# noway/nzcp-circom

Hardware: NVIDIA B200
Metric: groth16_proofs_per_sec (higher is better)
Workload: dtype u256 (Fr/Fq Montgomery, 8x32-bit limbs, IMAD.WIDE carry chains)

## Files before the change

nzcp_circom_b200/csrc/msm.cu:

```cuda
#include <atomic>

#include "common.cuh"
#include "msm_pair.cuh"

#ifndef NZCP_G2_ACC_BLOCKS
#define NZCP_G2_ACC_BLOCKS 3
#endif

namespace nzcp {

#ifndef NZCP_TASK_LEN_MAX
#define NZCP_TASK_LEN_MAX 64
#endif
static constexpr int kTaskLenMax = NZCP_TASK_LEN_MAX;
static_assert((NZCP_TASK_LEN_MAX & (NZCP_TASK_LEN_MAX - 1)) == 0 && NZCP_TASK_LEN_MAX >= 8, "task length must be a power of two");
static constexpr int kTaskLenMin = 8;
#ifndef NZCP_TARGET_TASKS
#define NZCP_TARGET_TASKS (148 * 640)
#endif
static constexpr int kTargetTasks = NZCP_TARGET_TASKS;
#ifndef NZCP_HEAVY_TASKS
#define NZCP_HEAVY_TASKS 16
#endif
static constexpr int kHeavyTasks = NZCP_HEAVY_TASKS;
// ... 275 lines not shown
#pragma unroll
  for (int r = 0; r < C; r++) carry[r] = 0;
  for (uint32_t base = 0; base < n_buckets; base += 4096) {
    const uint32_t b0 = base + threadIdx.x * 4;
    uint32_t v[C][4], sum[C], incl[C];
#pragma unroll
    for (int r = 0; r < C; r++) sum[r] = 0;
#pragma unroll
    for (int k = 0; k < 4; k++) {
      const uint32_t b = b0 + k;
      uint32_t len = b < n_buckets ? offsets[(size_t)(b + 1) * n_copies] - offsets[(size_t)b * n_copies] : 0u;
#pragma unroll
      for (int r = 0; r < C; r++) {
        v[r][k] = len;
        sum[r] += len;
        len = (len + 1) >> 1;
      }
      if (b < n_buckets) red_count[b] = v[R][k];
    }
#pragma unroll
    for (int r = 0; r < C; r++) {
      incl[r] = sum[r];
#pragma unroll
      for (int d = 1; d < 32; d <<= 1) {
        const uint32_t y = __shfl_up_sync(0xffffffffu, incl[r], d);
        if (lane >= (uint32_t)d) incl[r] += y;
      }
      if (lane == 31) wsum[r][warp] = incl[r];
    }
    __syncthreads();
    if (warp < (uint32_t)C) {
      const uint32_t w = wsum[warp][lane];
      uint32_t z = w;
#pragma unroll
      for (int d = 1; d < 32; d <<= 1) {
        const uint32_t y = __shfl_up_sync(0xffffffffu, z, d);
        if (lane >= (uint32_t)d) z += y;
      }
      wsum[warp][lane] = z - w;
      if (lane == 31) chunk_total[warp] = z;
    }
    __syncthreads();
#pragma unroll
    for (int r = 0; r < C; r++) {
      uint32_t run = carry[r] + wsum[r][warp] + (incl[r] - sum[r]);
#pragma unroll
      for (int k = 0; k < 4; k++) {
        if (b0 + k < n_buckets) round_off[(size_t)r * pitch + b0 + k] = run;
        run += v[r][k];
      }
      carry[r] += chunk_total[r];
    }
    __syncthreads();
  }
  if (threadIdx.x == 0) {
#pragma unroll
    for (int r = 0; r < C; r++) round_off[(size_t)r * pitch + n_buckets] = carry[r];
    flags[5] = carry[R];
  }
}

__global__ void __launch_bounds__(256)
msm_task_fill_kernel(const uint32_t* __restrict__ bcount, const uint32_t* __restrict__ offsets,
                     const uint32_t* __restrict__ task_off, uint2* __restrict__ tasks, uint32_t n_buckets,
                     const uint32_t* __restrict__ flags) {
  const uint32_t t = blockIdx.x * blockDim.x + threadIdx.x;
  if (t >= flags[2]) return;
  const uint32_t tl = flags[4];
  uint32_t lo = 0, hi = n_buckets;
  while (hi - lo > 1) {
    uint32_t mid = (lo + hi) >> 1;
    if (task_off[mid] <= t) lo = mid; else hi = mid;
  }
  (void)tl;
  const uint32_t k = task_off[lo + 1] - task_off[lo], j = t - task_off[lo];
  const uint32_t cnt = bcount[lo], base = cnt / k, rem = cnt % k;
  tasks[t] = make_uint2(offsets[lo] + j * base + (j < rem ? j : rem), base + (j < rem ? 1u : 0u));
}

template <class T>
__device__ __forceinline__ void prefetch_l1(const T* p) {
  asm volatile("prefetch.global.L1 [%0];" ::"l"(p));
  if (sizeof(T) > 64) asm volatile("prefetch.global.L1 [%0];" ::"l"(reinterpret_cast<const char*>(p) + 64));
}

template <class F> struct AccumOcc { static constexpr int kBlocks = 5; };
template <> struct AccumOcc<Fq2> { static constexpr int kBlocks = NZCP_G2_ACC_BLOCKS; };

template <class F>
__global__ void __launch_bounds__(128, AccumOcc<F>::kBlocks)
msm_accumulate_kernel(const Affine<F>* __restrict__ table, const uint32_t* __restrict__ entries,
                      const uint2* __restrict__ tasks, const uint32_t* __restrict__ flags, XYZZ<F>* __restrict__ partial, int pf) {
  uint32_t t = blockIdx.x * blockDim.x + threadIdx.x;
  if (t >= flags[2]) return;
  uint2 tk = tasks[t];
  XYZZ<F> acc = XYZZ<F>::inf();
  uint32_t e = entries[tk.x];
  if (pf & 1) prefetch_l1(table + (e & 0x7fffffffu));
  for (uint32_t k = 0; k < tk.y; k++) {
    uint32_t en = e;
    if (k + 1 < tk.y) {
      en = entries[tk.x + k + 1];
      if (pf & 1) prefetch_l1(table + (en & 0x7fffffffu));
    }
    Affine<F> q;
#if defined(__CUDA_ARCH__)
    if (sizeof(F) == sizeof(Fq) && (pf & 4)) q = gather_hinted<Affine<F>>(table + (e & 0x7fffffffu));
    else
#endif
      q = table[e & 0x7fffffffu];
    if (!q.is_inf()) xyzz_madd(acc, q, (e >> 31) != 0);
    e = en;
  }
  partial[t] = acc;
}

template <class F>
__global__ void __launch_bounds__(128, AccumOcc<F>::kBlocks)
msm_accumulate_pts_kernel(const Affine<F>* __restrict__ pts, const uint2* __restrict__ tasks,
                          const uint32_t* __restrict__ flags, XYZZ<F>* __restrict__ partial) {
  uint32_t t = blockIdx.x * blockDim.x + threadIdx.x;
  if (t >= flags[2]) return;
  uint2 tk = tasks[t];
  XYZZ<F> acc = XYZZ<F>::inf();
  for (uint32_t k = 0; k < tk.y; k++) {
    Affine<F> q = pts[tk.x + k];
    if (!q.is_inf()) xyzz_madd(acc, q, false);
  }
  partial[t] = acc;
}

static constexpr int kPairInvGroup = 32;
#ifndef NZCP_PAIR_FWD_BLOCKS
#define NZCP_PAIR_FWD_BLOCKS 1
#endif
template <class F, bool FROM_TABLE, int K>
__global__ void __launch_bounds__(128, (sizeof(F) == sizeof(Fq) ? NZCP_PAIR_FWD_BLOCKS : 1))
msm_pair_forward_kernel(const Affine<F>* __restrict__ src, const uint32_t* __restrict__ entries,
                        const uint32_t* __restrict__ off_in, const uint32_t* __restrict__ off_out, uint32_t n_buckets,
                        F* __restrict__ scratch, F* __restrict__ prod, int pf, Affine<F>* __restrict__ ops) {
  const uint32_t t = blockIdx.x * blockDim.x + threadIdx.x;
  PairSource<F, FROM_TABLE> ps{src, entries, pf};
  msm_pair_forward_body<F, FROM_TABLE, K>(t, gridDim.x * blockDim.x, ps, off_in, off_out, n_buckets, scratch, prod, ops);
}

template <class F, int K>
__global__ void __launch_bounds__(64)
msm_pair_invert_kernel(F* __restrict__ prod, const uint32_t* __restrict__ off_out, uint32_t n_buckets) {
  const uint32_t n_out = off_out[n_buckets];
  const uint32_t n_prod = pair_n_prod<K>(n_out);
  msm_pair_invert_body<F, kPairInvGroup>(blockIdx.x * blockDim.x + threadIdx.x, prod, n_prod);
}

template <class F, bool FROM_TABLE, int K>
__global__ void __launch_bounds__(128)
msm_pair_backward_kernel(const Affine<F>* __restrict__ src, const uint32_t* __restrict__ entries,
                         const uint32_t* __restrict__ off_in, const uint32_t* __restrict__ off_out, uint32_t n_buckets,
                         Affine<F>* __restrict__ dst, const F* __restrict__ scratch, const F* __restrict__ inv_prod, int pf,
                         const Affine<F>* __restrict__ ops) {
  const uint32_t t = blockIdx.x * blockDim.x + threadIdx.x;
  PairSource<F, FROM_TABLE> ps{src, entries, pf};
  msm_pair_backward_body<F, FROM_TABLE, K>(t, gridDim.x * blockDim.x, ps, off_in, off_out, n_buckets, dst, scratch, inv_prod,
                                           ops);
}

template <class T>
__device__ __forceinline__ T load_cg(const T* p) {
  static_assert(sizeof(T) % 16 == 0, "16-byte granules");
  T r;
  const uint4* s = reinterpret_cast<const uint4*>(p);
  uint4* d = reinterpret_cast<uint4*>(&r);
#pragma unroll
  for (int i = 0; i < (int)(sizeof(T) / 16); i++) d[i] = __ldcg(s + i);
  return r;
}

template <class T>
__device__ __forceinline__ T shfl_down_obj(const T& v, unsigned delta) {
  T r;
  const uint32_t* s = reinterpret_cast<const uint32_t*>(&v);
  uint32_t* d = reinterpret_cast<uint32_t*>(&r);
#pragma unroll
  for (int i = 0; i < (int)(sizeof(T) / 4); i++) d[i] = __shfl_down_sync(0xffffffffu, s[i], delta);
  return r;
}

template <class F>
__global__ void __launch_bounds__(128)
msm_combine_kernel(const uint32_t* __restrict__ task_off, const XYZZ<F>* __restrict__ partial,
                   XYZZ<F>* __restrict__ buckets, uint32_t n_buckets, uint32_t* __restrict__ heavy_list,
                   uint32_t* __restrict__ heavy_count) {
  const uint32_t b = blockIdx.x * blockDim.x + threadIdx.x;
  if (b >= n_buckets) return;
  const uint32_t t0 = task_off[b], nt = task_off[b + 1] - t0;
  if (nt > (uint32_t)kHeavyTasks) {
    heavy_list[atomicAdd(heavy_count, 1u)] = b;
    return;
  }
  XYZZ<F> acc = XYZZ<F>::inf();
  for (uint32_t j = 0; j < nt; j++) xyzz_add(acc, partial[t0 + j]);
  buckets[b] = acc;
}

__global__ void __launch_bounds__(1024)
msm_heavy_scan_kernel(const uint32_t* __restrict__ task_off, const uint32_t* __restrict__ heavy_list,
                      uint32_t* __restrict__ heavy_count, uint32_t* __restrict__ chunk_off) {
  __shared__ uint32_t sums[1024];
  const uint32_t n = heavy_count[0];
  const uint32_t per = (n + 1023) / 1024;
  const uint32_t b = threadIdx.x * per;
  const uint32_t e = b + per < n ? b + per : n;
  auto chunks = [&](uint32_t h) {
    uint32_t bk = heavy_list[h];
    return (task_off[bk + 1] - task_off[bk] + kHeavyChunk - 1) / kHeavyChunk;
  };
  uint32_t acc = 0;
  for (uint32_t h = b; h < e; h++) acc += chunks(h);
  sums[threadIdx.x] = acc;
  __syncthreads();
  for (int off = 1; off < 1024; off <<= 1) {
    uint32_t v = threadIdx.x >= (uint32_t)off ? sums[threadIdx.x - off] : 0;
    __syncthreads();
    sums[threadIdx.x] += v;
    __syncthreads();
  }
  uint32_t run = threadIdx.x ? sums[threadIdx.x - 1] : 0;
  for (uint32_t h = b; h < e; h++) {
    chunk_off[h] = run;
    run += chunks(h);
  }
  if (threadIdx.x == 1023) {
    chunk_off[n] = sums[1023];
    heavy_count[1] = sums[1023];
  }
}

template <class F>
__device__ __forceinline__ XYZZ<F> block_sum(XYZZ<F> acc, XYZZ<F>* sm) {
  sm[threadIdx.x] = acc;
  __syncthreads();
  for (uint32_t stride = blockDim.x / 2; stride >= 1; stride >>= 1) {
    if (threadIdx.x < stride) {
      XYZZ<F> a = sm[threadIdx.x];
      xyzz_add(a, sm[threadIdx.x + stride]);
      sm[threadIdx.x] = a;
    }
    __syncthreads();
  }
  XYZZ<F> r = sm[0];
  __syncthreads();
  return r;
}

template <class F>
__global__ void __launch_bounds__(kHeavyThreads)
msm_combine_heavy_kernel(const uint32_t* __restrict__ task_off, const XYZZ<F>* __restrict__ partial,
                         const uint32_t* __restrict__ heavy_list, const uint32_t* __restrict__ heavy_count,
                         const uint32_t* __restrict__ chunk_off, XYZZ<F>* __restrict__ chunk_partial,
                         XYZZ<F>* __restrict__ buckets) {
  extern __shared__ unsigned char heavy_sm_raw[];
  XYZZ<F>* sm = reinterpret_cast<XYZZ<F>*>(heavy_sm_raw);
  const uint32_t n_heavy = *heavy_count;
  const uint32_t total = chunk_off[n_heavy];
  for (uint32_t ch = blockIdx.x; ch < total; ch += gridDim.x) {
    uint32_t lo = 0, hi = n_heavy;
    while (hi - lo > 1) {
      uint32_t mid = (lo + hi) >> 1;
      if (chunk_off[mid] <= ch) lo = mid; else hi = mid;
    }
    const uint32_t b = heavy_list[lo];
    const uint32_t c = ch - chunk_off[lo];
    const uint32_t t0 = task_off[b] + c * kHeavyChunk;
    const uint32_t left = task_off[b + 1] - t0;
    const uint32_t cnt = left < (uint32_t)kHeavyChunk ? left : (uint32_t)kHeavyChunk;
    XYZZ<F> acc = XYZZ<F>::inf();
    for (uint32_t j = threadIdx.x; j < cnt; j += blockDim.x) xyzz_add(acc, partial[t0 + j]);
    acc = block_sum(acc, sm);
    if (threadIdx.x == 0) {
      if (chunk_off[lo + 1] - chunk_off[lo] == 1) buckets[b] = acc;
      else chunk_partial[ch] = acc;
    }
  }
}

template <class F>
__global__ void __launch_bounds__(kHeavyThreads)
msm_combine_heavy2_kernel(const uint32_t* __restrict__ heavy_list, const uint32_t* __restrict__ heavy_count,
                          const uint32_t* __restrict__ chunk_off, const XYZZ<F>* __restrict__ chunk_partial,
                          XYZZ<F>* __restrict__ buckets) {
  extern __shared__ unsigned char heavy_sm_raw[];
  XYZZ<F>* sm = reinterpret_cast<XYZZ<F>*>(heavy_sm_raw);
  const uint32_t n_heavy = *heavy_count;
  for (uint32_t h = blockIdx.x; h < n_heavy; h += gridDim.x) {
    const uint32_t c0 = chunk_off[h], nc = chunk_off[h + 1] - c0;
    if (nc <= 1) continue;
    XYZZ<F> acc = XYZZ<F>::inf();
    for (uint32_t j = threadIdx.x; j < nc; j += blockDim.x) xyzz_add(acc, chunk_partial[c0 + j]);
    acc = block_sum(acc, sm);
    if (threadIdx.x == 0) buckets[heavy_list[h]] = acc;
  }
}

static constexpr int kMargThreads = 128;

template <class F>
__device__ __forceinline__ XYZZ<F> warp_weighted_sum(XYZZ<F> run, uint32_t lane, XYZZ<F>* total) {
  for (uint32_t d = 1; d < 32; d <<= 1) {
    XYZZ<F> o = shfl_down_obj(run, d);
    if (lane + d < 32) xyzz_add(run, o);
  }
  *total = run;
  XYZZ<F> leaf = lane >= 1 ? run : XYZZ<F>::inf();
  for (uint32_t off = 16; off >= 1; off >>= 1) {
    XYZZ<F> o = shfl_down_obj(leaf, off);
    xyzz_add(leaf, o);
  }
// ... 187 lines not shown

void msm_sort_create(MsmSort* s, size_t n_points, int c, int rounds, bool table_free) {
  *s = MsmSort();
  if (c < 2 || c > 20) throw std::runtime_error("msm: window size out of range");
  s->n_points = n_points;
  s->c = c;
  s->rounds = rounds < 0 ? msm_pick_rounds(n_points, c) : (rounds > kMsmMaxRounds ? kMsmMaxRounds : rounds);
  s->n_windows = msm_num_windows(c);
  s->table_free = table_free;
  s->n_groups = table_free ? s->n_windows : 1;
  s->group_buckets = (size_t)1 << (c - 1);
  s->n_buckets = s->group_buckets * s->n_groups;
  if (s->n_buckets > ((size_t)1 << 19)) throw std::runtime_error("msm: too many buckets (window size too large for the table-free path)");
  size_t max_entries = (size_t)s->n_windows * n_points;
  if (max_entries >= ((size_t)1 << 31)) throw std::runtime_error("msm: too many points");
  size_t by_len = max_entries / kTaskLenMax, by_target = 2 * (size_t)kTargetTasks;
  if (max_entries / kTaskLenMin < by_target) by_target = max_entries / kTaskLenMin;
  s->max_tasks = s->n_buckets + (by_len > by_target ? by_len : by_target) + 1;
  size_t tot = 0;
  s->smem_hist = s->n_buckets <= (size_t)kSmemHistBuckets;
  s->n_copies = s->smem_hist ? 148 : kCopiesGlobal;
  size_t n_ctr = s->n_buckets * s->n_copies;
  s->counts = dev_alloc<uint32_t>(n_ctr + 1, &tot);
  s->offsets = dev_alloc<uint32_t>(n_ctr + 1, &tot);
  s->cursors = dev_alloc<uint32_t>(n_ctr + 1, &tot);
  s->red_count = dev_alloc<uint32_t>(s->n_buckets + 1, &tot);
  s->round_off = dev_alloc<uint32_t>((size_t)(kMsmMaxRounds + 1) * (s->n_buckets + 1), &tot);
  s->round_max[0] = max_entries;
  for (int r = 1; r <= kMsmMaxRounds; r++) s->round_max[r] = (s->round_max[r - 1] + s->n_buckets) / 2 + 1;
  s->block_sums = dev_alloc<uint32_t>(2 * (n_ctr / kScanBlock + 2), &tot);
  if (s->smem_hist) {
    NZCP_CUDA(cudaFuncSetAttribute(msm_digits_smem_kernel<false>, cudaFuncAttributeMaxDynamicSharedMemorySize, kSmemHistBuckets * 4));
    NZCP_CUDA(cudaFuncSetAttribute(msm_digits_smem_kernel<true>, cudaFuncAttributeMaxDynamicSharedMemorySize, kSmemHistBuckets * 4));
  }
  s->entries = dev_alloc<uint32_t>(max_entries, &tot);
  s->task_off = dev_alloc<uint32_t>(s->n_buckets + 1, &tot);
  s->tasks = dev_alloc<uint2>(s->max_tasks, &tot);
  s->flags = dev_alloc<uint32_t>(8, &tot);
  NZCP_CUDA(cudaMallocHost(&s->flags_host, 8 * sizeof(uint32_t)));
  memset(s->flags_host, 0, 8 * sizeof(uint32_t));
  s->scratch_bytes = tot;
}

void msm_sort_destroy(MsmSort* s) {
  cudaFree(s->counts);
  cudaFree(s->offsets);
  cudaFree(s->cursors);
  cudaFree(s->red_count);
  cudaFree(s->round_off);
  cudaFree(s->block_sums);
  cudaFree(s->entries);
  cudaFree(s->task_off);
  cudaFree(s->tasks);
  cudaFree(s->flags);
  if (s->flags_host) cudaFreeHost(s->flags_host);
  *s = MsmSort();
}

void msm_sort_launch(MsmSort* s, const Fr* scalars, size_t n_points, cudaStream_t st) {
  if (n_points > s->n_points) throw std::runtime_error("msm: sort plan too small");
  const uint32_t nb = (uint32_t)s->n_buckets;
  NZCP_CUDA(cudaMemsetAsync(s->flags, 0, 8 * sizeof(uint32_t), st));
  if (n_points) {
    uint32_t n_copies = s->n_copies;
    if (s->smem_hist) {
      uint32_t want = div_up(n_points, kSmemHistThreads);
      if (want < n_copies) n_copies = want;
    }
    int sort_threads = g_tune_sort_threads.load();
    sort_threads = sort_threads >= 1024 ? 1024 : sort_threads >= 512 ? 512 : sort_threads >= 256 ? 256 : 128;
    const uint32_t n_ctr = nb * n_copies;
    DigitParams dp{n_copies, (uint32_t)n_points, s->table_free ? 0u : (uint32_t)s->n_points, s->c, s->n_windows,
                   (uint32_t)s->group_buckets, s->table_free ? (uint32_t)s->group_buckets : 0u, nb};
    const unsigned gp = div_up(n_points, 256);
    const size_t hist_bytes = (size_t)nb * sizeof(uint32_t);
    if (s->smem_hist) {
      NZCP_CUDA(cudaMemsetAsync(s->counts + n_ctr, 0, sizeof(uint32_t), st));
      msm_digits_smem_kernel<false><<<n_copies, sort_threads, hist_bytes, st>>>(scalars, dp, s->counts, nullptr, s->flags);
    } else {
      NZCP_CUDA(cudaMemsetAsync(s->counts, 0, (n_ctr + 1) * sizeof(uint32_t), st));
      msm_digits_kernel<false><<<gp, 256, 0, st>>>(scalars, dp, s->counts, nullptr, s->flags);
    }
    NZCP_LAUNCH_CHECK();
    const uint32_t n_scan = n_ctr + 1;
    const uint32_t n_blk = div_up(n_scan, kScanBlock);
    uint32_t* blk_sum = s->block_sums;
    uint32_t* blk_off = s->block_sums + (s->n_buckets * s->n_copies / kScanBlock + 2);
    msm_scan_sums_kernel<<<n_blk, 256, 0, st>>>(s->counts, blk_sum, n_scan);
    NZCP_LAUNCH_CHECK();
    msm_scan_kernel<false><<<1, 1024, 0, st>>>(blk_sum, blk_off, n_blk, s->flags + 3, s->flags);
    NZCP_LAUNCH_CHECK();
    msm_scan_apply_kernel<<<n_blk, 256, 0, st>>>(s->counts, blk_off, s->offsets, s->smem_hist ? nullptr : s->cursors, n_scan);
    NZCP_LAUNCH_CHECK();
    if (s->smem_hist)
      msm_digits_smem_kernel<true><<<n_copies, sort_threads, hist_bytes, st>>>(scalars, dp, s->offsets, s->entries, s->flags);
    else
      msm_digits_kernel<true><<<gp, 256, 0, st>>>(scalars, dp, s->cursors, s->entries, s->flags);
    NZCP_LAUNCH_CHECK();
    switch (s->rounds) {
      case 0: msm_round_plan_kernel<0><<<1, 1024, 0, st>>>(s->offsets, n_copies, nb, s->round_off, s->red_count, s->flags); break;
      case 1: msm_round_plan_kernel<1><<<1, 1024, 0, st>>>(s->offsets, n_copies, nb, s->round_off, s->red_count, s->flags); break;
      case 2: msm_round_plan_kernel<2><<<1, 1024, 0, st>>>(s->offsets, n_copies, nb, s->round_off, s->red_count, s->flags); break;
      default: msm_round_plan_kernel<3><<<1, 1024, 0, st>>>(s->offsets, n_copies, nb, s->round_off, s->red_count, s->flags); break;
    }
    NZCP_LAUNCH_CHECK();
    msm_scan_kernel<true><<<1, 1024, 0, st>>>(s->red_count, s->task_off, nb, s->flags + 2, s->flags);
    NZCP_LAUNCH_CHECK();
    msm_task_fill_kernel<<<div_up(s->max_tasks, 256), 256, 0, st>>>(s->red_count, s->round_off + (size_t)s->rounds * (nb + 1),
                                                                     s->task_off, s->tasks, nb, s->flags);
    NZCP_LAUNCH_CHECK();
  } else {
    NZCP_CUDA(cudaMemsetAsync(s->task_off, 0, (nb + 1) * sizeof(uint32_t), st));
  }
  NZCP_CUDA(cudaMemcpyAsync(s->flags_host, s->flags, 8 * sizeof(uint32_t), cudaMemcpyDeviceToHost, st));
}

uint32_t msm_sort_check(const MsmSort* s) {
  if (s->flags_host[1]) throw std::runtime_error("witness/scalar value is not a canonical field element (>= r)");
  return s->flags_host[3];
}

void msm_run_create(MsmRun* r, const MsmSort* sort, bool g2) {
  *r = MsmRun();
  r->g2 = g2;
  size_t psz = g2 ? sizeof(G2XYZZ) : sizeof(G1XYZZ);
  size_t tot = 0;
  if (g2) {
    NZCP_CUDA(cudaFuncSetAttribute(msm_combine_heavy_kernel<Fq2>, cudaFuncAttributeMaxDynamicSharedMemorySize,
                                   (int)(kHeavyThreads * sizeof(G2XYZZ))));
    NZCP_CUDA(cudaFuncSetAttribute(msm_combine_heavy2_kernel<Fq2>, cudaFuncAttributeMaxDynamicSharedMemorySize,
                                   (int)(kHeavyThreads * sizeof(G2XYZZ))));
    NZCP_CUDA(cudaFuncSetAttribute(msm_marginal_kernel<Fq2>, cudaFuncAttributeMaxDynamicSharedMemorySize,
                                   (int)(kMargThreads * sizeof(G2XYZZ))));
  }
  r->partial = dev_alloc<unsigned char>(sort->max_tasks * psz, &tot);
  r->buckets = dev_alloc<unsigned char>(sort->n_buckets * psz, &tot);
  r->n_groups = sort->n_groups;
  r->c = sort->c;
  r->marg = dev_alloc<unsigned char>((size_t)r->n_groups * kMaxDigits * 32 * psz, &tot);
  r->marg_done = dev_alloc<uint32_t>((size_t)r->n_groups * kMaxDigits, &tot);
  NZCP_CUDA(cudaMemset(r->marg_done, 0, (size_t)r->n_groups * kMaxDigits * sizeof(uint32_t)));
  r->result = dev_alloc<unsigned char>(psz, &tot);
  r->heavy_list = dev_alloc<uint32_t>(sort->n_buckets, &tot);
  r->heavy_count = dev_alloc<uint32_t>(2, &tot);
  r->chunk_off = dev_alloc<uint32_t>(sort->n_buckets + 1, &tot);
  r->chunk_partial = dev_alloc<unsigned char>((sort->max_tasks / kHeavyChunk + sort->n_buckets + 1) * psz, &tot);
  r->out = dev_alloc<unsigned char>((size_t)r->n_groups * (kMaxDigits + 1) * psz, &tot);
  NZCP_CUDA(cudaMallocHost(&r->out_host, (size_t)r->n_groups * (kMaxDigits + 1) * psz));
  memset(r->out_host, 0, (size_t)r->n_groups * (kMaxDigits + 1) * psz);
  r->n_digits = (sort->c - 1 + 4) / 5;
  NZCP_CUDA(cudaFuncSetAttribute(msm_sum_points_kernel<Fq2>, cudaFuncAttributeMaxDynamicSharedMemorySize,
                                 (int)(kHeavyThreads * sizeof(G2XYZZ))));
  if (sort->rounds > 0) {
    const size_t asz = g2 ? sizeof(G2Affine) : sizeof(G1Affine), fsz = asz / 2, pad = 128 * 64;
    r->round_pts[0] = dev_alloc<unsigned char>((sort->round_max[1] + pad) * asz, &tot);
    if (sort->rounds > 1) r->round_pts[1] = dev_alloc<unsigned char>((sort->round_max[2] + pad) * asz, &tot);
    r->round_prefix = dev_alloc<unsigned char>((sort->round_max[1] + pad) * fsz, &tot);
    if (g_tune_pair_stage.load())
      r->round_ops = dev_alloc<unsigned char>((sort->round_max[1] + pad) * 2 * asz, &tot);
    r->round_prod = dev_alloc<unsigned char>((sort->round_max[1] / 4 + pad) * fsz, &tot);
  }
  NZCP_CUDA(cudaEventCreate(&r->ev_acc0));
  NZCP_CUDA(cudaEventCreate(&r->ev_acc1));
  r->scratch_bytes = tot;
}

void msm_run_destroy(MsmRun* r) {
  cudaFree(r->partial);
  cudaFree(r->buckets);
  cudaFree(r->marg);
  cudaFree(r->marg_done);
  cudaFree(r->result);
  cudaFree(r->heavy_list);
  cudaFree(r->heavy_count);
  cudaFree(r->chunk_off);
  cudaFree(r->chunk_partial);
  cudaFree(r->out);
  cudaFree(r->round_pts[0]);
  cudaFree(r->round_pts[1]);
  cudaFree(r->round_prefix);
  cudaFree(r->round_ops);
  cudaFree(r->round_prod);
  if (r->out_host) cudaFreeHost(r->out_host);
  if (r->ev_acc0) cudaEventDestroy(r->ev_acc0);
  if (r->ev_acc1) cudaEventDestroy(r->ev_acc1);
  *r = MsmRun();
}

template <class F>
static void msm_run_launch_t(MsmRun* r, const MsmSort* s, const MsmTable* t, cudaStream_t st) {
  if (t->c != s->c || t->n_points != s->n_points || t->n_windows != (s->table_free ? 1 : s->n_windows))
    throw std::runtime_error("msm: table and sort plan do not match");
  const uint32_t nb = (uint32_t)s->n_buckets;
  const size_t psz = sizeof(XYZZ<F>);
  XYZZ<F>* partial = reinterpret_cast<XYZZ<F>*>(r->partial);
  XYZZ<F>* buckets = reinterpret_cast<XYZZ<F>*>(r->buckets);
  XYZZ<F>* out = reinterpret_cast<XYZZ<F>*>(r->out);
  NZCP_CUDA(cudaMemsetAsync(r->heavy_count, 0, 2 * sizeof(uint32_t), st));
  NZCP_CUDA(cudaEventRecord(r->ev_acc0, st));
  if (s->rounds == 0) {
    msm_accumulate_kernel<F><<<div_up(s->max_tasks, 128), 128, 0, st>>>(reinterpret_cast<const Affine<F>*>(t->pts),
                                                                       s->entries, s->tasks, s->flags, partial,
                                                                       (g_tune_acc_prefetch.load() ? 1 : 0) | (g_tune_gather_hint.load() ? 4 : 0));
    NZCP_LAUNCH_CHECK();
  } else {
    const Affine<F>* src = reinterpret_cast<const Affine<F>*>(t->pts);
    for (int rd = 1; rd <= s->rounds; rd++) {
      Affine<F>* dst = reinterpret_cast<Affine<F>*>(r->round_pts[(rd - 1) & 1]);
      const uint32_t* off_in = s->round_off + (size_t)(rd - 1) * (nb + 1);
      const uint32_t* off_out = s->round_off + (size_t)rd * (nb + 1);
      const int hint = g_tune_gather_hint.load() ? 4 : 0;
      const int pf_fwd = g_tune_pair_prefetch[0].load() | hint, pf_bwd = g_tune_pair_prefetch[1].load() | hint;
      int k = g_tune_pair_k[rd - 1].load();
      k = k >= 32 ? 32 : k >= 16 ? 16 : k >= 8 ? 8 : 4;
      const unsigned grid = div_up(div_up(s->round_max[rd], k) + kPairLanes, 128);
      const unsigned grid_inv = div_up(div_up((size_t)grid * 128, kPairInvGroup), 64);
      F* scratch = reinterpret_cast<F*>(r->round_prefix);
      F* prod = reinterpret_cast<F*>(r->round_prod);
      Affine<F>* ops = g_tune_pair_stage.load() ? reinterpret_cast<Affine<F>*>(r->round_ops) : nullptr;
#define NZCP_PAIR_LAUNCH(TABLE, KK)                                                                                       \
      do {                                                                                                                \
        msm_pair_forward_kernel<F, TABLE, KK><<<grid, 128, 0, st>>>(src, s->entries, off_in, off_out, nb, scratch, prod, \
                                                                    pf_fwd, TABLE ? ops : nullptr);                       \
        NZCP_LAUNCH_CHECK();                                                                                              \
        msm_pair_invert_kernel<F, KK><<<grid_inv, 64, 0, st>>>(prod, off_out, nb);                                        \
        NZCP_LAUNCH_CHECK();                                                                                              \
        msm_pair_backward_kernel<F, TABLE, KK><<<grid, 128, 0, st>>>(src, s->entries, off_in, off_out, nb, dst, scratch,  \
                                                                     prod, pf_bwd, TABLE ? ops : nullptr);                \
        NZCP_LAUNCH_CHECK();                                                                                              \
      } while (0)
      if (rd == 1) {
        if (k == 32) NZCP_PAIR_LAUNCH(true, 32); else if (k == 16) NZCP_PAIR_LAUNCH(true, 16);
        else if (k == 8) NZCP_PAIR_LAUNCH(true, 8); else NZCP_PAIR_LAUNCH(true, 4);
      } else {
        if (k == 32) NZCP_PAIR_LAUNCH(false, 32); else if (k == 16) NZCP_PAIR_LAUNCH(false, 16);
        else if (k == 8) NZCP_PAIR_LAUNCH(false, 8); else NZCP_PAIR_LAUNCH(false, 4);
      }
#undef NZCP_PAIR_LAUNCH
      src = dst;
    }
    msm_accumulate_pts_kernel<F><<<div_up(s->max_tasks, 128), 128, 0, st>>>(src, s->tasks, s->flags, partial);
    NZCP_LAUNCH_CHECK();
  }
  NZCP_CUDA(cudaEventRecord(r->ev_acc1, st));
  msm_combine_kernel<F><<<div_up(nb, 128), 128, 0, st>>>(s->task_off, partial, buckets, nb, r->heavy_list,
                                                                     r->heavy_count);
  NZCP_LAUNCH_CHECK();
  msm_heavy_scan_kernel<<<1, 1024, 0, st>>>(s->task_off, r->heavy_list, r->heavy_count, r->chunk_off);
  NZCP_LAUNCH_CHECK();
  XYZZ<F>* chunk_partial = reinterpret_cast<XYZZ<F>*>(r->chunk_partial);
  msm_combine_heavy_kernel<F><<<148 * 16, kHeavyThreads, kHeavyThreads * psz, st>>>(s->task_off, partial, r->heavy_list,
                                                                                    r->heavy_count, r->chunk_off, chunk_partial,
                                                                                    buckets);
  NZCP_LAUNCH_CHECK();
  msm_combine_heavy2_kernel<F><<<148, kHeavyThreads, kHeavyThreads * psz, st>>>(r->heavy_list, r->heavy_count, r->chunk_off,
                                                                                chunk_partial, buckets);
  NZCP_LAUNCH_CHECK();
  const uint32_t bits = (uint32_t)(s->c - 1);
  const uint32_t n_digits = (bits + 4) / 5;
  XYZZ<F>* marg = reinterpret_cast<XYZZ<F>*>(r->marg);
  msm_marginal_kernel<F><<<(unsigned)s->n_groups * n_digits * 32, kMargThreads, kMargThreads * psz, st>>>(buckets, marg, out,
                                                                                                      r->marg_done, bits, n_digits);
  NZCP_LAUNCH_CHECK();
  NZCP_CUDA(cudaMemcpyAsync(r->out_host, r->out, (size_t)s->n_groups * (n_digits + 1) * psz, cudaMemcpyDeviceToHost, st));
}

void msm_run_finish_device(MsmRun* r, cudaStream_t st) {
  if (r->g2)
    msm_finish_kernel<Fq2><<<1, 32, 0, st>>>(reinterpret_cast<const G2XYZZ*>(r->out), reinterpret_cast<G2XYZZ*>(r->result),
                                             (uint32_t)r->n_groups, (uint32_t)r->n_digits, r->c);
  else
    msm_finish_kernel<Fq><<<1, 32, 0, st>>>(reinterpret_cast<const G1XYZZ*>(r->out), reinterpret_cast<G1XYZZ*>(r->result),
                                            (uint32_t)r->n_groups, (uint32_t)r->n_digits, r->c);
  NZCP_LAUNCH_CHECK();
}

void msm_sum_points(const void* d_pts, uint32_t count, bool g2, void* d_result, cudaStream_t st) {
  if (g2) {
    NZCP_CUDA(cudaFuncSetAttribute(msm_sum_points_kernel<Fq2>, cudaFuncAttributeMaxDynamicSharedMemorySize,
                                   (int)(kHeavyThreads * sizeof(G2XYZZ))));
    msm_sum_points_kernel<Fq2><<<1, kHeavyThreads, kHeavyThreads * sizeof(G2XYZZ), st>>>(
        reinterpret_cast<const G2XYZZ*>(d_pts), count, reinterpret_cast<G2XYZZ*>(d_result));
  } else {
    msm_sum_points_kernel<Fq><<<1, kHeavyThreads, kHeavyThreads * sizeof(G1XYZZ), st>>>(
        reinterpret_cast<const G1XYZZ*>(d_pts), count, reinterpret_cast<G1XYZZ*>(d_result));
  }
  NZCP_LAUNCH_CHECK();
}

void msm_run_launch(MsmRun* r, const MsmSort* sort, const MsmTable* table, cudaStream_t st) {
  if (r->g2 != table->g2) throw std::runtime_error("msm: run and table group mismatch");
  if (r->g2)
    msm_run_launch_t<Fq2>(r, sort, table, st);
  else
    msm_run_launch_t<Fq>(r, sort, table, st);
}

template <class F>
static XYZZ<F> msm_run_finish_t(const MsmRun* r) {
  XYZZ<F> res = XYZZ<F>::inf();
  for (int g = r->n_groups - 1; g >= 0; g--) {
    const XYZZ<F>* w = reinterpret_cast<const XYZZ<F>*>(r->out_host) + (size_t)g * (r->n_digits + 1);
    XYZZ<F> acc = XYZZ<F>::inf();
    for (int k = r->n_digits - 1; k >= 0; k--) {
      if (!acc.is_inf())
        for (int d = 0; d < 5; d++) acc = xyzz_dbl(acc);
      xyzz_add(acc, w[k]);
    }
    xyzz_add(acc, w[r->n_digits]);
    if (!res.is_inf())
      for (int d = 0; d < r->c; d++) res = xyzz_dbl(res);
    xyzz_add(res, acc);
  }
  return res;
}

G1XYZZ msm_run_finish_g1(const MsmRun* r) { return msm_run_finish_t<Fq>(r); }
G2XYZZ msm_run_finish_g2(const MsmRun* r) { return msm_run_finish_t<Fq2>(r); }

float msm_run_accumulate_ms(const MsmRun* r) {
  float ms = 0;
  if (cudaEventElapsedTime(&ms, r->ev_acc0, r->ev_acc1) != cudaSuccess) {
    cudaGetLastError();
    return 0;
  }
  return ms;
}

}
```

nzcp_circom_b200/csrc/msm_pair.cuh:

```cuda
#pragma once
#include "ec.cuh"


namespace nzcp {

enum PairKind { kPairNormal = 0, kPairDouble = 1, kPairFirst = 2, kPairSecond = 3, kPairInfinity = 4 };

#if defined(__CUDA_ARCH__)
template <class T>
__device__ __forceinline__ T gather_hinted(const T* p) {
  static_assert(sizeof(T) % 16 == 0, "16-byte granules");
  T r;
  uint4* d = reinterpret_cast<uint4*>(&r);
  const char* a = reinterpret_cast<const char*>(p);
#pragma unroll
  for (int i = 0; i < (int)(sizeof(T) / 16); i++)
    asm volatile("ld.global.nc.L2::64B.v4.u32 {%0, %1, %2, %3}, [%4];" : "=r"(d[i].x), "=r"(d[i].y), "=r"(d[i].z), "=r"(d[i].w) : "l"(a + 16 * i));
  return r;
}
#endif

template <class F, bool FROM_TABLE>
struct PairSource {
  const Affine<F>* pts;
  const uint32_t* entries;
  int pf = 0;
  HD uint32_t slot(uint32_t idx) const { return FROM_TABLE ? entries[idx] : idx; }
  HD F x_at(uint32_t slot) const {
#if defined(__CUDA_ARCH__)
    if (FROM_TABLE && (pf & 4)) return gather_hinted<F>(&pts[slot & 0x7fffffffu].x);
#endif
    return pts[FROM_TABLE ? (slot & 0x7fffffffu) : slot].x;
  }
  HD Affine<F> point_at(uint32_t slot) const {
    if (FROM_TABLE) {
      Affine<F> p;
#if defined(__CUDA_ARCH__)
      if (pf & 4) p = gather_hinted<Affine<F>>(&pts[slot & 0x7fffffffu]);
      else
#endif
        p = pts[slot & 0x7fffffffu];
      if (slot >> 31) p.y = f_neg(p.y);
      return p;
    }
    return pts[slot];
  }
  HD Affine<F> point(uint32_t idx) const { return point_at(slot(idx)); }
  HD void prefetch(uint32_t slot, bool whole_point) const {
#if defined(__CUDA_ARCH__)
    if ((pf & 3) == 0) return;
    const char* a = reinterpret_cast<const char*>(pts + (FROM_TABLE ? (slot & 0x7fffffffu) : slot));
    if ((pf & 3) == 1) {
      asm volatile("prefetch.global.L1 [%0];" ::"l"(a));
      if (sizeof(F) > 32 && whole_point) asm volatile("prefetch.global.L1 [%0];" ::"l"(a + 64));
    } else {
      asm volatile("prefetch.global.L2 [%0];" ::"l"(a));
      if (sizeof(F) > 32 && whole_point) asm volatile("prefetch.global.L2 [%0];" ::"l"(a + 64));
    }
#else
    (void)slot;
    (void)whole_point;
#endif
  }
};

struct PairWalk {
  const uint32_t* off_in;
  const uint32_t* off_out;
  uint32_t s, out0, out1, in0, len;
  HD void load() {
    out0 = off_out[s];
    out1 = off_out[s + 1];
    in0 = off_in[s];
    len = off_in[s + 1] - in0;
  }
  HD void forward_to(uint32_t o) {
    if (o < out1) return;
    do s++; while (o >= off_out[s + 1]);
    load();
  }
  HD void backward_to(uint32_t o) {
    if (o >= out0) return;
    do s--; while (o < off_out[s]);
    load();
  }
  HD uint32_t first(uint32_t o) const { return in0 + 2 * (o - out0); }
  HD bool paired(uint32_t o) const { return 2 * (o - out0) + 1 < len; }
};

template <class F>
HD int pair_classify(const Affine<F>& p1, const Affine<F>& p2, F& den) {
  if (p1.is_inf()) return kPairSecond;
  if (p2.is_inf()) return kPairFirst;
  den = f_sub(p2.x, p1.x);
  if (den.is_zero()) {
    if (p1.y == p2.y && !p1.y.is_zero()) {
      den = f_dbl(p1.y);
      return kPairDouble;
    }
    return kPairInfinity;
  }
  return kPairNormal;
}

static constexpr uint32_t kPairLanes = 32;
template <int K>
HD bool pair_thread_range(uint32_t t, const uint32_t* off_out, uint32_t n_buckets, uint32_t& o0, uint32_t& cnt) {
  const uint32_t n_out = off_out[n_buckets];
  const uint64_t first = (uint64_t)(t / kPairLanes) * (kPairLanes * K) + (t % kPairLanes);
  if (first >= n_out) return false;
  o0 = (uint32_t)first;
  const uint32_t left = (n_out - o0 + kPairLanes - 1) / kPairLanes;
  cnt = left < (uint32_t)K ? left : (uint32_t)K;
  return true;
}
template <int K>
HD uint32_t pair_n_prod(uint32_t n_out) {
  const uint32_t full = n_out / (kPairLanes * K), rem = n_out - full * (kPairLanes * K);
  return full * kPairLanes + (rem < kPairLanes ? rem : kPairLanes);
}
HD void pair_walk_seek(PairWalk& wk, uint32_t o, uint32_t n_buckets) {
  uint32_t lo = 0, hi = n_buckets;
  while (hi - lo > 1) {
    const uint32_t mid = (lo + hi) >> 1;
    if (wk.off_out[mid] <= o) lo = mid; else hi = mid;
  }
  wk.s = lo;
  wk.load();
}

template <class F, bool FROM_TABLE, int K>
HD void msm_pair_forward_body(uint32_t t, uint32_t stride, const PairSource<F, FROM_TABLE>& src, const uint32_t* off_in,
                              const uint32_t* off_out, uint32_t n_buckets, F* scratch, F* prod, Affine<F>* ops = nullptr) {
  uint32_t o0, cnt;
  if (!pair_thread_range<K>(t, off_out, n_buckets, o0, cnt)) return;
  PairWalk wk{off_in, off_out, 0, 0, 0, 0, 0};
  pair_walk_seek(wk, o0, n_buckets);
  F pre = F::one();
  bool have = false;
  bool pair_cur = wk.paired(o0);
  uint32_t a_cur = src.slot(wk.first(o0)), b_cur = pair_cur ? src.slot(wk.first(o0) + 1) : 0;
  for (uint32_t i = 0; i < cnt; i++) {
    bool pair_nxt = false;
    uint32_t a_nxt = 0, b_nxt = 0;
    if (i + 1 < cnt) {
      const uint32_t on = o0 + (i + 1) * kPairLanes;
      wk.forward_to(on);
      pair_nxt = wk.paired(on);
      if (pair_nxt || ops) a_nxt = src.slot(wk.first(on));
      if (pair_nxt) {
        b_nxt = src.slot(wk.first(on) + 1);
        src.prefetch(a_nxt, false);
        src.prefetch(b_nxt, false);
      }
    }
    if (ops) {
      const Affine<F> p1 = src.point_at(a_cur);
      const Affine<F> p2 = pair_cur ? src.point_at(b_cur) : Affine<F>::inf();
      ops[2 * ((size_t)i * stride + t)] = p1;
      ops[2 * ((size_t)i * stride + t) + 1] = p2;
      if (pair_cur) {
        F den;
        const int kind = pair_classify(p1, p2, den);
        if (kind == kPairNormal || kind == kPairDouble) {
          pre = have ? f_mul(pre, den) : den;
          have = true;
        }
      }
    } else if (pair_cur) {
      const F x1 = src.x_at(a_cur), x2 = src.x_at(b_cur);
      F den = f_sub(x2, x1);
      bool use = true;
      if (den.is_zero() || x1.is_zero() || x2.is_zero()) {
        const int kind = pair_classify(src.point_at(a_cur), src.point_at(b_cur), den);
        use = kind == kPairNormal || kind == kPairDouble;
      }
      if (use) {
        pre = have ? f_mul(pre, den) : den;
        have = true;
      }
    }
    scratch[(size_t)i * stride + t] = pre;
    pair_cur = pair_nxt;
    a_cur = a_nxt;
    b_cur = b_nxt;
  }
  prod[t] = pre;
}

template <class F, int KI>
HD void msm_pair_invert_body(uint32_t g, F* v, uint32_t n) {
  const uint32_t b = g * KI;
  if (b >= n) return;
  const uint32_t cnt = n - b < (uint32_t)KI ? n - b : (uint32_t)KI;
  F pre[KI];
  F run = v[b];
  pre[0] = run;
  for (uint32_t i = 1; i < cnt; i++) {
    run = f_mul(run, v[b + i]);
    pre[i] = run;
  }
  F inv = f_inv_fast(run);
  for (uint32_t i = cnt; i-- > 1;) {
    const F x = v[b + i];
    v[b + i] = f_mul(inv, pre[i - 1]);
    inv = f_mul(inv, x);
  }
  v[b] = inv;
}

template <class F>
HD Affine<F> pair_finish(const Affine<F>& p1, const Affine<F>& p2, F& inv, const F& before) {
  F den;
  const int kind = pair_classify(p1, p2, den);
  if (kind >= kPairFirst) return kind == kPairFirst ? p1 : kind == kPairSecond ? p2 : Affine<F>::inf();
  const F dinv = f_mul(inv, before);
  inv = f_mul(inv, den);
  F num;
  if (kind == kPairDouble) {
    const F xx = f_sqr(p1.x);
    num = f_add(f_dbl(xx), xx);
  } else {
    num = f_sub(p2.y, p1.y);
  }
  const F lam = f_mul(num, dinv);
  const F x3 = f_sub(f_sub(f_sqr(lam), p1.x), p2.x);
  const F y3 = f_sub(f_mul(lam, f_sub(p1.x, x3)), p1.y);
  return Affine<F>{x3, y3};
}

template <class F, bool FROM_TABLE, int K>
HD void msm_pair_backward_body(uint32_t t, uint32_t stride, const PairSource<F, FROM_TABLE>& src, const uint32_t* off_in,
                               const uint32_t* off_out, uint32_t n_buckets, Affine<F>* dst, const F* scratch,
                               const F* inv_prod, const Affine<F>* ops = nullptr) {
  uint32_t o0, cnt;
  if (!pair_thread_range<K>(t, off_out, n_buckets, o0, cnt)) return;
  if (ops) {
    F inv = inv_prod[t];
    for (uint32_t i = cnt; i-- > 0;) {
      const Affine<F> p1 = ops[2 * ((size_t)i * stride + t)], p2 = ops[2 * ((size_t)i * stride + t) + 1];
      const F before = i ? scratch[(size_t)(i - 1) * stride + t] : F::one();
      dst[o0 + i * kPairLanes] = pair_finish(p1, p2, inv, before);
    }
    return;
  }
  PairWalk wk{off_in, off_out, 0, 0, 0, 0, 0};
  pair_walk_seek(wk, o0 + (cnt - 1) * kPairLanes, n_buckets);
  F inv = inv_prod[t];
  bool pair_cur;
  uint32_t a_cur, b_cur;
  {
    const uint32_t o = o0 + (cnt - 1) * kPairLanes;
    pair_cur = wk.paired(o);
    a_cur = src.slot(wk.first(o));
    b_cur = pair_cur ? src.slot(wk.first(o) + 1) : 0;
  }
  for (uint32_t i = cnt; i-- > 0;) {
    const uint32_t o = o0 + i * kPairLanes;
    bool pair_nxt = false;
    uint32_t a_nxt = 0, b_nxt = 0;
    if (i > 0) {
      wk.backward_to(o - kPairLanes);
      pair_nxt = wk.paired(o - kPairLanes);
      a_nxt = src.slot(wk.first(o - kPairLanes));
      src.prefetch(a_nxt, true);
      if (pair_nxt) {
        b_nxt = src.slot(wk.first(o - kPairLanes) + 1);
        src.prefetch(b_nxt, true);
      }
    }
    if (!pair_cur) {
      dst[o] = src.point_at(a_cur);
    } else {
      const F before = i ? scratch[(size_t)(i - 1) * stride + t] : F::one();
      dst[o] = pair_finish(src.point_at(a_cur), src.point_at(b_cur), inv, before);
    }
    pair_cur = pair_nxt;
    a_cur = a_nxt;
    b_cur = b_nxt;
  }
}

}
```

Before: 131.7.

## Pipeline G2 pair backward gathers through a cp.async shared-memory ring

For Fq2 (G2), the backward pass of the pairwise affine-addition round now stages its loads in a per-thread, depth-2 shared-memory ring filled with cp.async. The loads are the bucket entry tags, the two gathered affine points and the prefix scratch value, so future items' loads overlap the current pair_finish arithmetic. The aim is to hide the latency of the random point gathers that stall the backward kernel. The cost is about 86KB of dynamic shared memory per 128-thread block, which may limit occupancy. It also adds extra shared-memory traffic and an extra tag-lookup stage; G1 keeps the old path.

New measurement: 131.9, median of 6. Within noise of the previous version (+0.2%).

```diff
diff --git a/nzcp_circom_b200/csrc/msm.cu b/nzcp_circom_b200/csrc/msm.cu
--- a/nzcp_circom_b200/csrc/msm.cu
+++ b/nzcp_circom_b200/csrc/msm.cu
@@ -451,8 +451,14 @@
   msm_pair_invert_body<F, kPairInvGroup>(blockIdx.x * blockDim.x + threadIdx.x, prod, n_prod);
 }
 
+template <class F>
+constexpr size_t pair_ring_bytes() {
+  constexpr int D = PairRingDepth<F>::kBackward;
+  if constexpr (D > 0) return kPairBlock * PairRing<D, 5 * (int)(sizeof(F) / 16)>::kThreadBytes;
+  else return 0;
+}
 template <class F, bool FROM_TABLE, int K>
-__global__ void __launch_bounds__(128)
+__global__ void __launch_bounds__(kPairBlock)
 msm_pair_backward_kernel(const Affine<F>* __restrict__ src, const uint32_t* __restrict__ entries,
                          const uint32_t* __restrict__ off_in, const uint32_t* __restrict__ off_out, uint32_t n_buckets,
                          Affine<F>* __restrict__ dst, const F* __restrict__ scratch, const F* __restrict__ inv_prod, int pf,
@@ -461,6 +467,22 @@
   PairSource<F, FROM_TABLE> ps{src, entries, pf};
   msm_pair_backward_body<F, FROM_TABLE, K>(t, gridDim.x * blockDim.x, ps, off_in, off_out, n_buckets, dst, scratch, inv_prod,
                                            ops);
+}
+
+template <bool TABLE, int K>
+static void pair_ring_attribute_k() {
+  NZCP_CUDA(cudaFuncSetAttribute(msm_pair_backward_kernel<Fq2, TABLE, K>, cudaFuncAttributeMaxDynamicSharedMemorySize,
+                                 (int)pair_ring_bytes<Fq2>()));
+}
+static void pair_ring_attributes() {
+  pair_ring_attribute_k<true, 4>();
+  pair_ring_attribute_k<true, 8>();
+  pair_ring_attribute_k<true, 16>();
+  pair_ring_attribute_k<true, 32>();
+  pair_ring_attribute_k<false, 4>();
+  pair_ring_attribute_k<false, 8>();
+  pair_ring_attribute_k<false, 16>();
+  pair_ring_attribute_k<false, 32>();
 }
 
 template <class T>
@@ -954,6 +976,7 @@
   NZCP_CUDA(cudaFuncSetAttribute(msm_sum_points_kernel<Fq2>, cudaFuncAttributeMaxDynamicSharedMemorySize,
                                  (int)(kHeavyThreads * sizeof(G2XYZZ))));
   if (sort->rounds > 0) {
+    if (g2) pair_ring_attributes();
     const size_t asz = g2 ? sizeof(G2Affine) : sizeof(G1Affine), fsz = asz / 2, pad = 128 * 64;
     r->round_pts[0] = dev_alloc<unsigned char>((sort->round_max[1] + pad) * asz, &tot);
     if (sort->rounds > 1) r->round_pts[1] = dev_alloc<unsigned char>((sort->round_max[2] + pad) * asz, &tot);
@@ -1027,7 +1050,8 @@
         NZCP_LAUNCH_CHECK();                                                                                              \
         msm_pair_invert_kernel<F, KK><<<grid_inv, 64, 0, st>>>(prod, off_out, nb);                                        \
         NZCP_LAUNCH_CHECK();                                                                                              \
-        msm_pair_backward_kernel<F, TABLE, KK><<<grid, 128, 0, st>>>(src, s->entries, off_in, off_out, nb, dst, scratch,  \
+        msm_pair_backward_kernel<F, TABLE, KK><<<grid, kPairBlock, pair_ring_bytes<F>(), st>>>(src, s->entries, off_in,  \
+                                                                     off_out, nb, dst, scratch,                           \
                                                                      prod, pf_bwd, TABLE ? ops : nullptr);                \
         NZCP_LAUNCH_CHECK();                                                                                              \
       } while (0)
diff --git a/nzcp_circom_b200/csrc/msm_pair.cuh b/nzcp_circom_b200/csrc/msm_pair.cuh
--- a/nzcp_circom_b200/csrc/msm_pair.cuh
+++ b/nzcp_circom_b200/csrc/msm_pair.cuh
@@ -1,4 +1,6 @@
 #pragma once
+#include <string.h>
+
 #include "ec.cuh"
 
 
@@ -46,6 +48,11 @@
     return pts[slot];
   }
   HD Affine<F> point(uint32_t idx) const { return point_at(slot(idx)); }
+  HD const Affine<F>* at(uint32_t slot) const { return pts + (FROM_TABLE ? (slot & 0x7fffffffu) : slot); }
+  HD Affine<F> signed_point(Affine<F> p, uint32_t slot) const {
+    if (FROM_TABLE && (slot >> 31)) p.y = f_neg(p.y);
+    return p;
+  }
   HD void prefetch(uint32_t slot, bool whole_point) const {
 #if defined(__CUDA_ARCH__)
     if ((pf & 3) == 0) return;
@@ -229,6 +236,126 @@
   return Affine<F>{x3, y3};
 }
 
+template <class F> struct PairRingDepth { static constexpr int kBackward = 0; };
+template <> struct PairRingDepth<Fq2> { static constexpr int kBackward = 2; };
+
+static constexpr int kPairBlock = 128;
+
+template <int D, int W>
+struct PairRing {
+  static constexpr int kTags = 2 * D;
+  static constexpr size_t kThreadBytes = (size_t)D * W * 16 + (size_t)kTags * 8;
+#if defined(__CUDA_ARCH__)
+  uint4* g;
+  uint2* tg;
+  HD PairRing() {
+    extern __shared__ uint4 pair_ring_smem[];
+    g = pair_ring_smem + threadIdx.x;
+    tg = reinterpret_cast<uint2*>(pair_ring_smem + D * W * kPairBlock) + threadIdx.x;
+  }
+  HD void fetch(uint32_t s, int w, const void* src, int n) {
+    const uint4* p = static_cast<const uint4*>(src);
+#pragma unroll
+    for (int k = 0; k < n; k++) {
+      const uint32_t d = (uint32_t)__cvta_generic_to_shared(g + (s * W + w + k) * kPairBlock);
+      asm volatile("cp.async.ca.shared.global [%0], [%1], 16;" ::"r"(d), "l"(p + k) : "memory");
+    }
+  }
+  HD void fetch_tag(uint32_t u, const uint32_t* e, bool two) {
+    const uint32_t d = (uint32_t)__cvta_generic_to_shared(tg + u * kPairBlock);
+    asm volatile("cp.async.ca.shared.global [%0], [%1], 4;" ::"r"(d), "l"(e) : "memory");
+    if (two) asm volatile("cp.async.ca.shared.global [%0], [%1], 4;" ::"r"(d + 4), "l"(e + 1) : "memory");
+  }
+  HD void set_tag(uint32_t u, uint32_t a, uint32_t b) { tg[u * kPairBlock] = make_uint2(a, b); }
+  HD uint2 tag(uint32_t u) const { return tg[u * kPairBlock]; }
+  template <class T>
+  HD T get(uint32_t s, int w) const {
+    T r;
+    uint4* d = reinterpret_cast<uint4*>(&r);
+#pragma unroll
+    for (int k = 0; k < (int)(sizeof(T) / 16); k++) d[k] = g[(s * W + w + k) * kPairBlock];
+    return r;
+  }
+  HD void commit() { asm volatile("cp.async.commit_group;" ::: "memory"); }
+  HD void wait() { asm volatile("cp.async.wait_group %0;" ::"n"(D - 1) : "memory"); }
+  HD void wait_all() { asm volatile("cp.async.wait_group 0;" ::: "memory"); }
+#else
+  uint4 g[D * W];
+  uint2 tg[kTags];
+  HD void fetch(uint32_t s, int w, const void* src, int n) { memcpy(&g[s * W + w], src, 16 * (size_t)n); }
+  HD void fetch_tag(uint32_t u, const uint32_t* e, bool two) { tg[u] = make_uint2(e[0], two ? e[1] : 0u); }
+  HD void set_tag(uint32_t u, uint32_t a, uint32_t b) { tg[u] = make_uint2(a, b); }
+  HD uint2 tag(uint32_t u) const { return tg[u]; }
+  template <class T>
+  HD T get(uint32_t s, int w) const {
+    T r;
+    memcpy(&r, &g[s * W + w], sizeof(T));
+    return r;
+  }
+  HD void commit() {}
+  HD void wait() {}
+  HD void wait_all() {}
+#endif
+};
+
+template <int D, class Ring, class Look, class Issue, class Compute>
+HD void pair_pipeline(Ring& ring, uint32_t cnt, Look look, Issue issue, Compute compute) {
+  for (uint32_t q = 0; q < (uint32_t)D && q < cnt; q++) look(q);
+  ring.commit();
+  ring.wait_all();
+  for (uint32_t q = 0; q < (uint32_t)D; q++) {
+    if (q < cnt) issue(q);
+    if (q + D < cnt) look(q + D);
+    ring.commit();
+  }
+  for (uint32_t q = 0; q < cnt; q++) {
+    ring.wait();
+    compute(q);
+    if (q + D < cnt) issue(q + D);
+    if (q + 2 * D < cnt) look(q + 2 * D);
+    ring.commit();
+  }
+}
+
+template <class F, bool FROM_TABLE>
+HD void msm_pair_backward_ring(uint32_t t, uint32_t stride, const PairSource<F, FROM_TABLE>& src, PairWalk& wk,
+                               uint32_t o0, uint32_t cnt, Affine<F>* dst, const F* scratch, F inv) {
+  constexpr int D = PairRingDepth<F>::kBackward, G = (int)(sizeof(F) / 16);
+  PairRing<D, 5 * G> ring;
+  uint32_t paired = 0;
+  pair_pipeline<D>(
+      ring, cnt,
+      [&](uint32_t q) {
+        const uint32_t o = o0 + (cnt - 1 - q) * kPairLanes;
+        wk.backward_to(o);
+        const bool two = wk.paired(o);
+        paired |= (uint32_t)two << q;
+        if (FROM_TABLE) ring.fetch_tag(q % (2 * D), src.entries + wk.first(o), two);
+        else ring.set_tag(q % (2 * D), wk.first(o), wk.first(o) + 1);
+      },
+      [&](uint32_t q) {
+        const uint32_t i = cnt - 1 - q;
+        const uint2 sl = ring.tag(q % (2 * D));
+        ring.fetch(q % D, 0, src.at(sl.x), 2 * G);
+        if ((paired >> q) & 1) {
+          ring.fetch(q % D, 2 * G, src.at(sl.y), 2 * G);
+          if (i) ring.fetch(q % D, 4 * G, scratch + (size_t)(i - 1) * stride + t, G);
+        }
+      },
+      [&](uint32_t q) {
+        const uint32_t i = cnt - 1 - q;
+        const uint2 sl = ring.tag(q % (2 * D));
+        const Affine<F> p1 = src.signed_point(ring.template get<Affine<F>>(q % D, 0), sl.x);
+        if (!((paired >> q) & 1)) {
+          dst[o0 + i * kPairLanes] = p1;
+        } else {
+          const Affine<F> p2 = src.signed_point(ring.template get<Affine<F>>(q % D, 2 * G), sl.y);
+          const F before = i ? ring.template get<F>(q % D, 4 * G) : F::one();
+          dst[o0 + i * kPairLanes] = pair_finish(p1, p2, inv, before);
+        }
+      });
+}
+
 template <class F, bool FROM_TABLE, int K>
 HD void msm_pair_backward_body(uint32_t t, uint32_t stride, const PairSource<F, FROM_TABLE>& src, const uint32_t* off_in,
                                const uint32_t* off_out, uint32_t n_buckets, Affine<F>* dst, const F* scratch,
@@ -247,6 +374,10 @@
   PairWalk wk{off_in, off_out, 0, 0, 0, 0, 0};
   pair_walk_seek(wk, o0 + (cnt - 1) * kPairLanes, n_buckets);
   F inv = inv_prod[t];
+  if constexpr (PairRingDepth<F>::kBackward > 0) {
+    msm_pair_backward_ring<F, FROM_TABLE>(t, stride, src, wk, o0, cnt, dst, scratch, inv);
+    return;
+  }
   bool pair_cur;
   uint32_t a_cur, b_cur;
   {
```
